# HongwenZhang/DaNet-DensePose2SMPL

Measured on AMD Instinct MI355X. Metric: images/sec fwd+bwd HRNet-W48+SMPL+IUV 256x256 bs32/GPU, higher is better.
Workload: dtype bf16; 1 GPU; full DaNet train step (HRNet-W48 + global and part-wise IUV heads + regressor nets + SMPL LBS (2 forward + 1 backward; the 2 label-side forwards belong to the untimed batch prologue) + IUV render + losses, fwd+bwd+Adam), 256x256, 32 img/GPU; convs bf16 MFMA fp32-acc, LBS/raster/losses fp32; global_batch=32, parallelism=dp1

## Files before the change

### danet-densepose2smpl_amd/_lib.py

```python
import ctypes
import os

_HERE = os.path.dirname(os.path.abspath(__file__))
LIB_PATH = os.environ.get('DANET_LIB') or os.path.join(_HERE, 'csrc', 'libdanet_hip.so')
_lib = None

c_f = ctypes.c_void_p
c_i = ctypes.c_int
c_sz = ctypes.c_size_t
c_fl = ctypes.c_float

_SIGNATURES = {
    'danet_version': (c_i, []),
    'danet_last_error': (ctypes.c_char_p, []),
    'danet_smpl_lbs_debug': (c_i, [c_f]),
    'danet_smpl_lbs_ctx_floats': (c_sz, [c_i]),
    'danet_smpl_lbs_fwd_ws_floats': (c_sz, [c_i, c_i, c_i]),
    'danet_smpl_lbs_bwd_ws_floats': (c_sz, [c_i, c_i, c_i]),
    'danet_smpl_lbs_ticket_words': (c_sz, [c_i]),
    'danet_smpl_lbs_forward': (c_i, [c_f, c_f, c_i] + [c_f] * 9 + [c_i] * 4 + [c_f] * 5 + [c_sz, c_f, c_f]),
    'danet_smpl_lbs_backward': (c_i, [c_f, c_f, c_i] + [c_f] * 7 + [c_i] * 4 + [c_f] * 7 + [c_sz, c_f, c_i, c_f]),
    'danet_smpl_lbs_backward_fused_ok': (c_i, [c_i, c_i, c_i]),
    'danet_iuv_raster_ws_bytes': (c_sz, [c_i, c_i, c_i]),
    'danet_iuv_raster_forward': (c_i, [c_f, c_f, c_i, c_i, c_f, c_i, c_f, c_f, c_i, c_fl, c_fl, c_i, c_f, c_f, c_f, c_f, c_sz, c_f]),
# ... 133 lines not shown


class BnBwdJob(ctypes.Structure):
    _fields_ = [(k, ctypes.c_void_p) for k in ('dy', 'x', 'y', 'gamma', 'saved', 'dx', 'dres', 'dparam', 'red', 'beta', 'mask')] + \
               [('M', ctypes.c_int64), ('C', c_i), ('red_state', c_i), ('relu', c_i), ('mask_mode', c_i)]


class GcnLayer(ctypes.Structure):
    _fields_ = [(k, ctypes.c_void_p) for k in ('W', 'bias', 'gamma', 'beta', 'running_mean', 'running_var')]


class GcnTailArgs(ctypes.Structure):
    _fields_ = [('x', ctypes.c_void_p), ('L', GcnLayer * 5)] + \
               [(k, ctypes.c_void_p) for k in ('A_r2p', 'A_p2r', 'A_mask', 'edge')] + \
               [('Wp', ctypes.c_void_p * 2), ('bp', ctypes.c_void_p * 2), ('Wc', ctypes.c_void_p * 2), ('bc', ctypes.c_void_p * 2)] + \
               [(k, ctypes.c_void_p) for k in ('mean_pose', 'ws', 'jr0', 'jp0', 'jp1', 'pose', 'g_jr0', 'g_jp0', 'g_jp1', 'g_pose', 'gx')] + \
               [('gW', ctypes.c_void_p * 5), ('gb', ctypes.c_void_p * 5), ('ggamma', ctypes.c_void_p * 5), ('gbeta', ctypes.c_void_p * 5),
                ('gedge', ctypes.c_void_p),
                ('gWp', ctypes.c_void_p * 2), ('gbp', ctypes.c_void_p * 2), ('gWc', ctypes.c_void_p * 2), ('gbc', ctypes.c_void_p * 2),
                ('scratch', ctypes.c_void_p), ('bar', ctypes.c_void_p), ('B', c_i), ('momentum', ctypes.c_float), ('eps', ctypes.c_float)]


class ConvJob(ctypes.Structure):
    _fields_ = [(k, ctypes.c_void_p) for k in ('x', 'wp', 'y', 'bn_sums', 'bn_x', 'bn_y', 'bn_saved', 'bn_red', 'addend')] + \
               [(k, c_i) for k in ('B', 'H', 'W', 'Cin', 'OH', 'OW', 'Cout', 'R', 'S', 'stride', 'pad', 'dil', 'groups', 'transposed', 'bn_gate')]


def exported_symbols():
    return list(_SIGNATURES)


KNOBS = {'c3_enable': 1, 'c3_mt': 2, 'c3_kw': 3, 'c3_blocks': 4, 'c3_want': 5, 'c3s_enable': 6, 'c3s_blocks': 7, 'c3s_kw': 8, 'c3s_want': 9,
         'pw': 10, 'pw_wgrad': 11, 'stem': 12, 'stem_dgrad': 13, 'c3a': 14, 'bn_block_bytes': 15,
         'c3s_balance': 16, 'c3s_tile_cost': 17, 'g3': 18}


class _Library(object):

    def __init__(self, cdll):
        self._cdll = cdll

    def __getattr__(self, name):
        return getattr(self._cdll, name)

    def knob(self, name, value=-1):
        return int(self._cdll.danet_knob(KNOBS[name], int(value)))

    def danet_conv3x3_set(self, enable, force_mt, force_kw, blocks, want_tiles):
        prev = self.knob('c3_enable', enable)
        if force_mt >= 0 and force_kw >= 0:
            self.knob('c3_mt', force_mt)
            self.knob('c3_kw', force_kw)
        self.knob('c3_blocks', blocks if blocks > 0 else -1)
        self.knob('c3_want', want_tiles)
        return prev

    def danet_conv3x3_stream_set(self, enable, blocks, kw, want_tiles):
        prev = self.knob('c3s_enable', enable)
        self.knob('c3s_blocks', blocks if blocks > 0 else -1)
        self.knob('c3s_kw', kw)
        self.knob('c3s_want', want_tiles)
        return prev

    def danet_conv_pw_set(self, enable):
        return self.knob('pw', enable)

    def danet_conv_pw_wgrad_set(self, enable):
# ... 68 lines not shown
```

### danet-densepose2smpl_amd/csrc/capi.hip

```cpp
#include "common.h"
#include "conv_common.h"

namespace danet {
char* last_error_buf() {
    static thread_local char buf[kErrLen] = {0};
    return buf;
}

namespace {
__global__ __launch_bounds__(256) void zero_kernel(unsigned* __restrict__ p, size_t n4, size_t tail0, size_t n) {
    uint4* const q = reinterpret_cast<uint4*>(p);
    for (size_t i = (size_t)blockIdx.x * 256 + threadIdx.x; i < n4; i += (size_t)gridDim.x * 256) q[i] = uint4{0u, 0u, 0u, 0u};
    for (size_t i = tail0 + (size_t)blockIdx.x * 256 + threadIdx.x; i < n; i += (size_t)gridDim.x * 256) p[i] = 0u;
}
}

hipError_t zero_async(void* p, size_t bytes, hipStream_t stream) {
    if (bytes == 0) return hipSuccess;
    if ((bytes & 3) || (reinterpret_cast<size_t>(p) & 3)) return hipErrorInvalidValue;
    const size_t n = bytes / 4;
    const bool al16 = (reinterpret_cast<size_t>(p) & 15) == 0;
    const size_t n4 = al16 ? n / 4 : 0, tail0 = n4 * 4;
    size_t blocks = ((al16 ? n4 : n) + 255) / 256;
    if (blocks > 2048) blocks = 2048;
    if (blocks < 1) blocks = 1;
    hipLaunchKernelGGL(zero_kernel, dim3((unsigned)blocks), dim3(256), 0, stream, (unsigned*)p, n4, tail0, n);
    return hipGetLastError();
}
}

extern "C" int danet_version(void) { return 100; }

extern "C" long danet_knob(int id, long value) {
    using namespace danet_conv;
    switch (id) {
        case DANET_KNOB_C3_ENABLE: case DANET_KNOB_C3_MT: case DANET_KNOB_C3_KW: case DANET_KNOB_C3_BLOCKS: case DANET_KNOB_C3_WANT:
            return conv3x3_knob(id, value);
        case DANET_KNOB_C3S_ENABLE: case DANET_KNOB_C3S_BLOCKS: case DANET_KNOB_C3S_KW: case DANET_KNOB_C3S_WANT:
        case DANET_KNOB_C3S_BALANCE: case DANET_KNOB_C3S_TILE_COST:
            return conv3x3s_knob(id, value);
        case DANET_KNOB_PW: return conv_pw_knob(value);
        case DANET_KNOB_PW_WGRAD: return conv_pw_wgrad_knob(value);
        case DANET_KNOB_STEM: return conv_stem_knob(value);
        case DANET_KNOB_STEM_DGRAD: return conv_stem_dgrad_knob(value);
        case DANET_KNOB_C3A: return conv3x3a_knob(value);
        case DANET_KNOB_G3: return conv_g3_knob(value);
        case DANET_KNOB_BN_BLOCK_BYTES: return bn_block_bytes_knob(value);
        default: return -1;
    }
}
extern "C" const char* danet_last_error(void) { return danet::last_error_buf(); }
```

### danet-densepose2smpl_amd/csrc/conv_common.h

```cpp
#pragma once
#include <hip/hip_runtime.h>

namespace danet_conv {

typedef unsigned short bf16_t;
typedef __attribute__((ext_vector_type(8))) __bf16 bf16x8;
typedef __attribute__((ext_vector_type(4))) float f32x4;

typedef __attribute__((ext_vector_type(2))) float f32x2_;
typedef __attribute__((ext_vector_type(2))) __bf16 bf16x2_;
__device__ inline unsigned f2bf_pk(float lo, float hi) {
    return __builtin_bit_cast(unsigned, __builtin_convertvector(f32x2_{lo, hi}, bf16x2_));
}
__device__ inline bf16_t f2bf(float f) { return (bf16_t)(f2bf_pk(f, 0.f) & 0xffffu); }
__device__ inline float bf2f(bf16_t h) { return __uint_as_float((unsigned)h << 16); }

constexpr int BN_NCOPY = 32;
#ifndef DANET_BN_NCOPY_DIV
#define DANET_BN_NCOPY_DIV 2
#endif
__host__ __device__ inline int bn_ncopy(int C) {
    const int n = (C <= 64 ? 32 : (C <= 128 ? 16 : (C <= 256 ? 8 : 4))) / DANET_BN_NCOPY_DIV;
    return n < 4 ? 4 : n;
}
// ... 34 lines not shown
    const bf16_t* addend;
    const BnApply* bna;
};


bool conv_fast_ok(const ConvP& p, bool vec8, int mt);
int conv_fast_launch(const ConvP& p, int mt, int nt, void* stream);
int conv_fast_launch_multi(const ConvP* ps, const int* mts, int n, int nt, void* stream);

bool conv_pw_ok(const ConvP& p, bool vec8);
int conv_pw_config(const ConvP& p);
int conv_pw_launch(const ConvP& p, void* stream);

struct WgJob { const void* x; const void* dy; float* dw; int B, H, W, Cin, OH, OW, Cout, R, S, stride, pad, dil, groups; };
bool conv_pw_wgrad_ok(const WgJob& j);
size_t conv_pw_wgrad_ws_floats(const WgJob* jobs, const int* idx, int cnt, long target);
int conv_pw_wgrad_launch(const WgJob* jobs, const int* idx, int cnt, float* ws, float beta, long target, void* stream);

bool conv_g3_ok(const ConvP& p, bool vec8);
int conv_g3_launch(const ConvP& p, void* stream);

bool conv3x3_ok(const ConvP& p, bool vec8);
int conv3x3_config(const ConvP& p, bool vec8, int nprob);
int conv3x3_launch(const ConvP* ps, int n, void* stream, bool dry = false);

int conv3x3s_launch(const ConvP* ps, int n, void* stream, bool dry);
bool conv3x3_stream_first();
int* conv3x3_debug_buffer();

long conv3x3_knob(int id, long value);
long conv3x3s_knob(int id, long value);
long conv_pw_knob(long value);
long conv_pw_wgrad_knob(long value);
long conv_stem_knob(long value);
long conv_stem_dgrad_knob(long value);
long conv3x3a_knob(long value);
long conv_g3_knob(long value);
long bn_block_bytes_knob(long value);

}
```

### danet-densepose2smpl_amd/csrc/conv_wgrad3x3.hip

```cpp
#include <cstdlib>
#include "common.h"
#include "conv_common.h"

namespace {

using namespace danet_conv;

constexpr int TH = 4, TW = 8;
constexpr int halo_h(int st) { return st * (TH - 1) + 3; }
constexpr int halo_w(int st) { return st * (TW - 1) + 3; }

struct Wg3P {
    const bf16_t* x; const bf16_t* dy; float* part;
    float* direct;
    int B, H, W, Cin, Cout, groups, Cin_g, Cout_g;
    int IH, IW;
    int tiles_h, tiles_w, msplit;
    long nchunks;
    long x_bytes, dy_bytes;
};

typedef __attribute__((ext_vector_type(2))) unsigned v2u;

__device__ inline v2u tr_read(unsigned lds_byte_addr) {
    v2u r;
    asm volatile("ds_read_b64_tr_b16 %0, %1" : "=v"(r) : "v"(lds_byte_addr) : "memory");
    return r;
}

template <int CT, int NI, int ST, int SM = 0>
__device__ __forceinline__ void wgrad3x3_body(const Wg3P& p, const int bx, const int by, const int bz)
{
    constexpr bool PAIR = SM != 0;
    constexpr int OS = SM ? SM : 4;
    constexpr int PHW = ST * (OS - 1) + 3;
    constexpr int IMH = SM ? TH / OS : 1, IMW = SM ? TW / OS : 1;
    constexpr int HH = SM ? IMH * PHW : halo_h(ST), HW = SM ? IMW * PHW : halo_w(ST);
    constexpr int HALF = SM ? (4 / OS) * PHW : ST * 4;
    constexpr int BCO = CT * 16, BCI = NI * 16;
    constexpr int PXY = BCO * 2, PXX = BCI * 2;
    extern __shared__ __attribute__((aligned(16))) unsigned char smem[];
    constexpr int YB = TH * TW * PXY, XB = HH * HW * PXX, BUF = YB + XB;

    const int t = threadIdx.x, lane = t & 63, wave = t >> 6;
    const int li = lane & 15, lg = lane >> 4;
    const int nci = (p.Cin_g + BCI - 1) / BCI;
    const int cib = by % nci, cob = by / nci;
    const int g = bz;
    const int co0 = cob * BCO, ci0 = cib * BCI;
    const bf16_t* const dyg = p.dy + (size_t)g * p.Cout_g + co0;
    const bf16_t* const xg = p.x + (size_t)g * p.Cin_g + ci0;

    constexpr int NPAIR = 9 * NI;
    constexpr int MAXP = (NPAIR + 3) / 4;
    f32x4 acc[MAXP][CT];
    unsigned boff[MAXP];
#pragma unroll
    for (int pi = 0; pi < MAXP; ++pi) {
#pragma unroll
        for (int ct = 0; ct < CT; ++ct) acc[pi][ct] = f32x4{0.f, 0.f, 0.f, 0.f};
        const int pair = min(wave + 4 * pi, NPAIR - 1);
        const int tap = pair / NI, ni = pair - tap * NI;
        const int r = tap / 3, s = tap - r * 3;
        const int hrow = SM ? (lg / OS) * PHW + ST * (lg % OS) + r : ST * lg + r;
        const int hcol = SM ? ((li >> 2) / OS) * PHW + ST * ((li >> 2) % OS) + s : ST * (li >> 2) + s;
        boff[pi] = (unsigned)((hrow * HW + hcol) * PXX + (ni * 16 + 4 * (li & 3)) * 2);
    }
    const unsigned aoff = (unsigned)((lg * TW + (li >> 2)) * PXY + (4 * (li & 3)) * 2);

    const int nchunks = (int)p.nchunks;
    const int per = (nchunks + p.msplit - 1) / p.msplit;
    const int c_begin = bx * per, c_end = min(nchunks, c_begin + per);

    constexpr int NPY = TH * TW * (BCO / 8), NPX = HH * HW * (BCI / 8);
    constexpr int NRY = (NPY + 255) / 256, NRX = (NPX + 255) / 256;
    constexpr int OOB = 0x7fffffff;
    const __amdgpu_buffer_rsrc_t yr = __builtin_amdgcn_make_buffer_rsrc(const_cast<bf16_t*>(dyg), 0, (int)p.dy_bytes, 0x00020000);
    const __amdgpu_buffer_rsrc_t xr = __builtin_amdgcn_make_buffer_rsrc(const_cast<bf16_t*>(xg), 0, (int)p.x_bytes, 0x00020000);
    int yrel[NRY], xrel[NRX], xhy[NRX], xhx[NRX];
#pragma unroll
    for (int u = 0; u < NRY; ++u) {
        const int pc = t + u * 256;
        const int c8 = pc % (BCO / 8), q = pc / (BCO / 8);
        const int ty = q / TW, tx = q % TW;
        const int ypix = SM ? ((ty / OS) * IMW + tx / OS) * (OS * OS) + (ty % OS) * OS + tx % OS : ty * p.W + tx;
        yrel[u] = (pc < NPY && co0 + c8 * 8 < p.Cout_g) ? (ypix * p.Cout + c8 * 8) * 2 : OOB;
    }
#pragma unroll
    for (int u = 0; u < NRX; ++u) {
        const int pc = t + u * 256;
        const int c8 = pc % (BCI / 8), q = pc / (BCI / 8);
        const bool live = pc < NPX && ci0 + c8 * 8 < p.Cin_g;
        if (PAIR) {
            const int hq = q / HW, img = (hq / PHW) * IMW + (q % HW) / PHW, hy = hq % PHW - 1, hc = (q % HW) % PHW - 1;
            const bool inside = live && (unsigned)hy < (unsigned)(OS * ST) && (unsigned)hc < (unsigned)(OS * ST);
            xrel[u] = ((img * (OS * OS * ST * ST) + hy * (OS * ST) + hc) * p.Cin + c8 * 8) * 2;
            xhy[u] = inside ? 1 : -100000;
            xhx[u] = 1;
        } else {
            xrel[u] = (((q / HW - 1) * p.IW + q % HW - 1) * p.Cin + c8 * 8) * 2;
            xhy[u] = live ? q / HW : -100000;
            xhx[u] = q % HW;
        }
    }
    int f_tw = c_begin % p.tiles_w, f_th = (c_begin / p.tiles_w) % p.tiles_h, f_b = c_begin / (p.tiles_w * p.tiles_h);
    uint4 ystage[NRY], xstage[NRX];

    auto fetch = [&]() {
        const int oh0 = f_th * TH, ow0 = f_tw * TW;
        const int pix0 = (f_b * p.H + oh0) * p.W + ow0;
        const int by = pix0 * p.Cout * 2, bx = ((f_b * p.IH + ST * oh0) * p.IW + ST * ow0) * p.Cin * 2;
#pragma unroll
        for (int u = 0; u < NRY; ++u)
            ystage[u] = __builtin_bit_cast(uint4, __builtin_amdgcn_raw_buffer_load_b128(yr, yrel[u] != OOB ? by + yrel[u] : OOB, 0, 0));
#pragma unroll
        for (int u = 0; u < NRX; ++u) {
            const bool ok = PAIR ? xhy[u] > 0
                                 : ((unsigned)(ST * oh0 - 1 + xhy[u]) < (unsigned)p.IH && (unsigned)(ST * ow0 - 1 + xhx[u]) < (unsigned)p.IW);
            xstage[u] = __builtin_bit_cast(uint4, __builtin_amdgcn_raw_buffer_load_b128(xr, ok ? bx + xrel[u] : OOB, 0, 0));
        }
        if (++f_tw == p.tiles_w) { f_tw = 0; if (++f_th == p.tiles_h) { f_th = 0; ++f_b; } }
    };
    auto commit = [&](int buf) {
        unsigned char* base = smem + buf * BUF;
#pragma unroll
        for (int u = 0; u < NRY; ++u)
            if (t + u * 256 < NPY) *reinterpret_cast<uint4*>(base + (size_t)(t + u * 256) * 16) = ystage[u];
#pragma unroll
        for (int u = 0; u < NRX; ++u)
            if (t + u * 256 < NPX) *reinterpret_cast<uint4*>(base + (size_t)(NPY + t + u * 256) * 16) = xstage[u];
    };

    if (c_begin < c_end) fetch();
    int buf = 0;
    for (int ch = c_begin; ch < c_end; ++ch) {
        commit(buf);
        __syncthreads();
        if (ch + 1 < c_end) fetch();
        const unsigned ybase = (unsigned)(buf * BUF), xbase = ybase + YB;
        v2u alo[CT], ahi[CT], blo[MAXP], bhi[MAXP];
#pragma unroll
        for (int ct = 0; ct < CT; ++ct) {
            alo[ct] = tr_read(ybase + aoff + ct * 32);
            ahi[ct] = tr_read(ybase + aoff + ct * 32 + 4 * PXY);
        }
#pragma unroll
        for (int pi = 0; pi < MAXP; ++pi) {
            blo[pi] = tr_read(xbase + boff[pi]);
            bhi[pi] = tr_read(xbase + boff[pi] + HALF * PXX);
        }
        asm volatile("s_waitcnt lgkmcnt(0)" ::: "memory");
        __builtin_amdgcn_sched_barrier(0);
        bf16x8 a[CT];
#pragma unroll
        for (int ct = 0; ct < CT; ++ct) {
            const uint4 raw = {alo[ct].x, alo[ct].y, ahi[ct].x, ahi[ct].y};
            a[ct] = __builtin_bit_cast(bf16x8, raw);
        }
#pragma unroll
        for (int pi = 0; pi < MAXP; ++pi) {
            const uint4 raw = {blo[pi].x, blo[pi].y, bhi[pi].x, bhi[pi].y};
            const bf16x8 bq = __builtin_bit_cast(bf16x8, raw);
#pragma unroll
            for (int ct = 0; ct < CT; ++ct)
                acc[pi][ct] = __builtin_amdgcn_mfma_f32_16x16x32_bf16(a[ct], bq, acc[pi][ct], 0, 0, 0);
        }
        buf ^= 1;
    }
    const int gsz = 9 * p.Cout_g * p.Cin_g;
    if (p.direct) {
        float* const dw = p.direct + (size_t)g * gsz;
#pragma unroll
        for (int pi = 0; pi < MAXP; ++pi) {
            const int pair = wave + 4 * pi;
            const int tap = pair / NI, ni = pair - tap * NI;
            const int cin = ci0 + ni * 16 + li;
            if (pair >= NPAIR || cin >= p.Cin_g) continue;
#pragma unroll
            for (int ct = 0; ct < CT; ++ct)
#pragma unroll
                for (int r = 0; r < 4; ++r) {
                    const int cout = co0 + ct * 16 + lg * 4 + r;
                    if (cout < p.Cout_g) dw[((size_t)cout * p.Cin_g + cin) * 9 + tap] = acc[pi][ct][r];
                }
        }
        return;
    }
    float* dst = p.part + ((size_t)bx * p.groups + g) * gsz;
#pragma unroll
    for (int pi = 0; pi < MAXP; ++pi) {
        const int pair = wave + 4 * pi;
        const int tap = pair / NI, ni = pair - tap * NI;
        const int cin = ci0 + ni * 16 + li;
        if (pair >= NPAIR || cin >= p.Cin_g) continue;
        float* row = dst + ((tap * p.Cout_g + co0 + lg * 4) * p.Cin_g + cin);
#pragma unroll
        for (int ct = 0; ct < CT; ++ct)
#pragma unroll
            for (int r = 0; r < 4; ++r)
                if (co0 + ct * 16 + lg * 4 + r < p.Cout_g) row[(ct * 16 + r) * p.Cin_g] = acc[pi][ct][r];
    }
}

template <int CT, int NI, int ST>
__global__ __launch_bounds__(256) void conv_wgrad3x3_kernel(Wg3P p)
{
    wgrad3x3_body<CT, NI, ST>(p, blockIdx.x, blockIdx.y, blockIdx.z);
}

constexpr int NPM = 20;
struct Wg3Multi { Wg3P p[NPM]; int start[NPM + 1]; int nyb[NPM]; int n; int xcd; };

template <int CT, int NI, int ST, int SM = 0>
__global__ __launch_bounds__(256) void conv_wgrad3x3_multi_kernel(Wg3Multi mp)
{
    int vb = (int)blockIdx.x;
    if (mp.xcd) {
        const int G = (int)gridDim.x, q = G >> 3, r = G & 7;
        const int x = vb & 7, slot = vb >> 3;
        vb = x * q + (x < r ? x : r) + slot;
    }
    int i = 0;
    while (i + 1 < mp.n && vb >= mp.start[i + 1]) ++i;
    const int l = vb - mp.start[i];
    const Wg3P& p = mp.p[i];
    const int bx = l % p.msplit, rest = l / p.msplit;
    wgrad3x3_body<CT, NI, ST, SM>(p, bx, rest % mp.nyb[i], rest / mp.nyb[i]);
}

struct Red3Multi { const float* part[NPM]; float* dw[NPM]; int G[NPM], Cout_g[NPM], Cin_g[NPM], msplit[NPM]; long start[NPM + 1]; int n; float beta; };

__global__ __launch_bounds__(256) void wgrad3x3_reduce_multi_kernel(Red3Multi rp)
{
    const long gidx = (long)blockIdx.x * 256 + threadIdx.x;
    if (gidx >= rp.start[rp.n]) return;
    int i = 0;
    while (i + 1 < rp.n && gidx >= rp.start[i + 1]) ++i;
    const long idx = gidx - rp.start[i], total = rp.start[i + 1] - rp.start[i];
    const float* part = rp.part[i];
    float s = 0.f;
    int sp = 0;
    for (; sp + 4 <= rp.msplit[i]; sp += 4) {
        const float v0 = part[(size_t)sp * total + idx], v1 = part[(size_t)(sp + 1) * total + idx];
        const float v2 = part[(size_t)(sp + 2) * total + idx], v3 = part[(size_t)(sp + 3) * total + idx];
        s += (v0 + v1) + (v2 + v3);
    }
    for (; sp < rp.msplit[i]; ++sp) s += part[(size_t)sp * total + idx];
    const int Cin_g = rp.Cin_g[i], Cout_g = rp.Cout_g[i];
    const int cin = (int)(idx % Cin_g);
    long rest = idx / Cin_g;
    const int cout = (int)(rest % Cout_g); rest /= Cout_g;
    const int tap = (int)(rest % 9), g = (int)(rest / 9);
    const size_t o = (((size_t)(g * Cout_g + cout)) * Cin_g + cin) * 9 + tap;
    float* dw = rp.dw[i];
    dw[o] = rp.beta != 0.f ? dw[o] * rp.beta + s : s;
}

__global__ __launch_bounds__(256) void wgrad3x3_reduce_kernel(const float* __restrict__ part, float* __restrict__ dw,
                                                               int G, int Cout_g, int Cin_g, int msplit, float beta)
{
    const long total = (long)G * Cout_g * Cin_g * 9;
    const long idx = (long)blockIdx.x * 256 + threadIdx.x;
    if (idx >= total) return;
    float s = 0.f;
    int sp = 0;
    for (; sp + 4 <= msplit; sp += 4) {
        const float v0 = part[(size_t)sp * total + idx], v1 = part[(size_t)(sp + 1) * total + idx];
        const float v2 = part[(size_t)(sp + 2) * total + idx], v3 = part[(size_t)(sp + 3) * total + idx];
        s += (v0 + v1) + (v2 + v3);
    }
    for (; sp < msplit; ++sp) s += part[(size_t)sp * total + idx];
    const int cin = (int)(idx % Cin_g);
    long rest = idx / Cin_g;
    const int cout = (int)(rest % Cout_g); rest /= Cout_g;
    const int tap = (int)(rest % 9), g = (int)(rest / 9);
    const size_t o = (((size_t)(g * Cout_g + cout)) * Cin_g + cin) * 9 + tap;
    dw[o] = beta != 0.f ? dw[o] * beta + s : s;
}

template <int CT, int NI, int ST>
int launch3(const Wg3P& p, hipStream_t st) {
    const int nco = (p.Cout_g + CT * 16 - 1) / (CT * 16), nci = (p.Cin_g + NI * 16 - 1) / (NI * 16);
    const size_t lds = 2 * (size_t)(TH * TW * CT * 32 + halo_h(ST) * halo_w(ST) * NI * 32);
    hipLaunchKernelGGL((conv_wgrad3x3_kernel<CT, NI, ST>), dim3(p.msplit, nco * nci, p.groups), dim3(256), lds, st, p);
    return 0;
}

inline int tiles3(int c) { return c <= 16 ? 1 : (c <= 32 ? 2 : ((c % 48 == 0 || c <= 48) ? 3 : 4)); }

}

extern "C" int danet_conv_wgrad3x3_ok(int H, int W, int Cin, int Cout, int R, int S, int stride, int pad, int dil, int groups) {
    static const bool no_s2 = getenv("DANET_NO_WGRAD3_S2") != nullptr;
    if (!(R == 3 && S == 3 && (stride == 1 || (stride == 2 && !no_s2)) && pad == 1 && dil == 1)) return 0;
    if (H % stride != 0 || W % stride != 0) return 0;
    return (H / stride) % TH == 0 && (W / stride) % TW == 0 && (Cin / groups) % 8 == 0 && (Cout / groups) % 8 == 0;
}

extern "C" int danet_conv_wgrad3x3_pair_ok(int B, int H, int W, int Cin, int Cout, int R, int S, int stride, int pad, int dil, int groups) {
    static const bool off = getenv("DANET_NO_WGRAD3_PAIR") != nullptr;
    if (off || !(R == 3 && S == 3 && (stride == 1 || stride == 2) && pad == 1 && dil == 1 && H == W && B > 0 && groups > 0)) return 0;
    if (!((H == 4 * stride && B % 2 == 0) || (H == 2 * stride && B % 8 == 0))) return 0;
    if (Cin % groups != 0 || Cout % groups != 0) return 0;
    const int ci = Cin / groups, co = Cout / groups;
    if (ci % 8 != 0 || co % 8 != 0) return 0;
    return 1;
}
static inline int wg3_small(int B, int H, int W, int stride) {
    if (!(stride == 1 || stride == 2) || H != W) return 0;
    if (H == 4 * stride && B % 2 == 0) return 4;
    if (H == 2 * stride && B % 8 == 0) return 2;
    return 0;
}
static inline bool wg3_is_pair(int B, int H, int W, int stride) { return wg3_small(B, H, W, stride) != 0; }

static void plan3(int B, int H, int W, int Cin, int Cout, int groups, int* ct, int* ni, int* msplit) {
    const int Cout_g = Cout / groups, Cin_g = Cin / groups;
    *ct = tiles3(Cout_g); *ni = tiles3(Cin_g);
    if (*ct == 4) *ct = 2;
    if (*ni == 4) *ni = 2;
    const long other = (long)((Cout_g + *ct * 16 - 1) / (*ct * 16)) * ((Cin_g + *ni * 16 - 1) / (*ni * 16)) * groups;
    const long nchunks = (long)B * (H / TH) * (W / TW);
// ... 111 lines not shown
        int msplit[NPM];
        plan_multi(jobs, idx, cnt, ct, ni, msplit);
        Wg3Multi mp; Red3Multi rp;
        static const bool xcd_order = getenv("DANET_WGRAD3_XCD") && atoi(getenv("DANET_WGRAD3_XCD")) != 0;
        mp.n = cnt; rp.n = cnt; rp.beta = beta; mp.xcd = xcd_order ? 1 : 0;
        mp.start[0] = 0; rp.start[0] = 0;
        for (int k = 0; k < cnt; ++k) {
            const Wg3Job& j = jobs[idx[k]];
            Wg3P& p = mp.p[k];
            static const bool no_direct = getenv("DANET_WGRAD3_NO_DIRECT") != nullptr;
            const bool direct = msplit[k] == 1 && beta == 0.f && !no_direct;
            p.x = (const bf16_t*)j.x; p.dy = (const bf16_t*)j.dy; p.part = (ws && !direct) ? ws + used : nullptr;
            p.direct = direct ? j.dw : nullptr;
            p.IH = j.H; p.IW = j.W;
            p.B = j.B; p.H = j.H / stride; p.W = j.W / stride; p.Cin = j.Cin; p.Cout = j.Cout; p.groups = j.groups;
            if (pair) { p.B = j.B / (sm == 4 ? 2 : 8); p.H = 4; p.W = 8; p.IH = 4 * stride; p.IW = 8 * stride; }
            p.Cin_g = j.Cin / j.groups; p.Cout_g = j.Cout / j.groups;
            p.tiles_h = p.H / TH; p.tiles_w = p.W / TW;
            p.nchunks = (long)p.B * p.tiles_h * p.tiles_w;
            p.x_bytes = (long)j.B * j.H * j.W * j.Cin * 2; p.dy_bytes = (long)j.B * (j.H / stride) * (j.W / stride) * j.Cout * 2;
            p.msplit = msplit[k];
            const int nyb = ((p.Cout_g + ct * 16 - 1) / (ct * 16)) * ((p.Cin_g + ni * 16 - 1) / (ni * 16));
            mp.nyb[k] = nyb;
            mp.start[k + 1] = mp.start[k] + msplit[k] * nyb * j.groups;
            const long total = (long)j.Cout * p.Cin_g * 9;
            rp.part[k] = p.part; rp.dw[k] = j.dw; rp.G[k] = j.groups; rp.Cout_g[k] = p.Cout_g; rp.Cin_g[k] = p.Cin_g; rp.msplit[k] = msplit[k];
            rp.start[k + 1] = rp.start[k] + (direct ? 0 : total);
            if (!direct || !ws) used += (size_t)msplit[k] * total;
            if (ws && !(p.x_bytes < (1L << 31) && p.dy_bytes < (1L << 31)))
                return danet::fail(DANET_ERR_ARG, "conv_wgrad3x3_multi: tensors of 2 GB or more are not supported");
        }
        if (!ws) continue;
        if (used > ws_floats) return danet::fail(DANET_ERR_WORKSPACE, "conv_wgrad3x3_multi: workspace too small");
        const int phw = stride * ((sm ? sm : 4) - 1) + 3;
        const size_t lds = 2 * (size_t)(TH * TW * ct * 32 + (sm ? (TH / sm) * phw * (TW / sm) * phw : halo_h(stride) * halo_w(stride)) * ni * 32);
        const dim3 grid((unsigned)mp.start[cnt]);
        if (pair) {
#define W3P(a, b) if (ct == a && ni == b) { \
            if (stride == 1 && sm == 4) hipLaunchKernelGGL((conv_wgrad3x3_multi_kernel<a, b, 1, 4>), grid, dim3(256), lds, st, mp); \
            else if (stride == 2 && sm == 4) hipLaunchKernelGGL((conv_wgrad3x3_multi_kernel<a, b, 2, 4>), grid, dim3(256), lds, st, mp); \
            else if (stride == 1) hipLaunchKernelGGL((conv_wgrad3x3_multi_kernel<a, b, 1, 2>), grid, dim3(256), lds, st, mp); \
            else hipLaunchKernelGGL((conv_wgrad3x3_multi_kernel<a, b, 2, 2>), grid, dim3(256), lds, st, mp); } else
            W3P(2, 2) W3P(2, 3) W3P(3, 2) W3P(3, 3) W3P(1, 1) W3P(1, 2) W3P(2, 1) W3P(1, 3) W3P(3, 1)
            return danet::fail(DANET_ERR_ARG, "conv_wgrad3x3_multi: no pair-mode kernel for tiles %dx%d", ct, ni);
#undef W3P
        } else
#define W3M(a, b) if (ct == a && ni == b) { \
            if (stride == 1) hipLaunchKernelGGL((conv_wgrad3x3_multi_kernel<a, b, 1>), grid, dim3(256), lds, st, mp); \
            else hipLaunchKernelGGL((conv_wgrad3x3_multi_kernel<a, b, 2>), grid, dim3(256), lds, st, mp); } else
        W3M(1, 1) W3M(1, 2) W3M(1, 3) W3M(2, 1) W3M(2, 2) W3M(2, 3) W3M(3, 1) W3M(3, 2) W3M(3, 3)
        return danet::fail(DANET_ERR_ARG, "conv_wgrad3x3_multi: no kernel for tiles %dx%d", ct, ni);
#undef W3M
        DANET_CHECK_LAUNCH("conv_wgrad3x3_multi_kernel");
        if (rp.start[cnt] > 0) {
            hipLaunchKernelGGL(wgrad3x3_reduce_multi_kernel, dim3((unsigned)danet::cdiv(rp.start[cnt], 256)), dim3(256), 0, st, rp);
            DANET_CHECK_LAUNCH("wgrad3x3_reduce_multi_kernel");
        }
    }
    if (need_out) *need_out = used;
    return DANET_OK;
}

extern "C" size_t danet_conv_wgrad3x3_multi_ws_floats(const void* jobs, int n)
{
    size_t need = 0;
    if (!jobs || n <= 0) return 0;
    multi_foreach_launch((const Wg3Job*)jobs, n, nullptr, 0, 0.f, nullptr, &need);
    return need;
}

extern "C" int danet_conv_wgrad3x3_multi(const void* jobs, int n, float* ws, size_t ws_floats, float beta, void* stream)
{
    DANET_ENTER();
    DANET_CHECK_ARG(jobs && n > 0 && ws, "conv_wgrad3x3_multi: bad arguments");
    const Wg3Job* jb = (const Wg3Job*)jobs;
    for (int i = 0; i < n; ++i)
        DANET_CHECK_ARG(jb[i].x && jb[i].dy && jb[i].dw && jb[i].B > 0 &&
                        (danet_conv_wgrad3x3_ok(jb[i].H, jb[i].W, jb[i].Cin, jb[i].Cout, 3, 3, jb[i].stride, 1, 1, jb[i].groups) ||
                         danet_conv_wgrad3x3_pair_ok(jb[i].B, jb[i].H, jb[i].W, jb[i].Cin, jb[i].Cout, 3, 3, jb[i].stride, 1, 1, jb[i].groups)),
                        "conv_wgrad3x3_multi: job %d is not a supported 3x3 problem", i);
    return multi_foreach_launch(jb, n, ws, ws_floats, beta, (hipStream_t)stream, nullptr);
}
// ... 1 lines not shown
```

### include/danet_hip.h

```cpp
#ifndef DANET_HIP_H
#define DANET_HIP_H

#include <stddef.h>
#include <stdint.h>

#ifdef __cplusplus
extern "C" {
#endif

#define DANET_OK 0
#define DANET_ERR_ARG (-1)
#define DANET_ERR_HIP (-2)
#define DANET_ERR_WORKSPACE (-3)

int danet_version(void);
const char* danet_last_error(void);

size_t danet_smpl_lbs_ctx_floats(int B);
size_t danet_smpl_lbs_fwd_ws_floats(int B, int V, int NE);
size_t danet_smpl_lbs_bwd_ws_floats(int B, int V, int NB);
size_t danet_smpl_lbs_ticket_words(int B);

int danet_smpl_lbs_forward(const float* betas, const float* rotmats, int B,
                           const float* v_template, const float* shapedirs, const float* posedirs,
// ... 106 lines not shown
int danet_conv_pack_weights_padded(const float* w, void* wp, int Cout, int Cin_g, int R, int S, int groups,
                                   int mode, int chunk, int src_Cout_g, int src_Cin_g, void* stream);
long danet_conv_pack_job_fill_padded(void* job_host, const float* w, void* wp, long start, long bstart,
                                     int Cout, int Cin_g, int R, int S, int groups, int mode, int chunk, int src_Cout_g, int src_Cin_g);
size_t danet_conv_pack_job_bytes(void);
long danet_conv_pack_job_bricks(int Cout, int Cin_g, int R, int S, int groups, int mode, int chunk);
long danet_conv_pack_job_fill(void* job_host, const float* w, void* wp, long start, long bstart,
                              int Cout, int Cin_g, int R, int S, int groups, int mode, int chunk);
int danet_conv_pack_weights_batched(const void* jobs_dev, int njobs, long total_elems, long total_bricks, void* stream);
int danet_conv_f32(int mode, const float* a, const float* b, const float* bias, float* out,
                   int B, int H, int W, int Cin, int OH, int OW, int Cout, int R, int S, int stride, int pad, int dil, int groups,
                   void* stream);
size_t danet_conv_f32m_packed_elems(int Cout_gp, int Cin_gp, int R, int S, int groups, int mode);
int danet_conv_f32m_pack_weights(const float* w, float* wp, int Cout, int Cin_g, int R, int S, int groups, int mode,
                                 int Cout_gp, int Cin_gp, void* stream);
int danet_conv_f32m_ok(int B, int H, int W, int Cin, int OH, int OW, int Cout, int R, int S, int stride, int pad, int dil,
                       int groups, int transposed);
int danet_conv_f32m_forward(const float* x, const float* wp, const float* bias, float* y,
                            int B, int H, int W, int Cin, int OH, int OW, int Cout, int R, int S, int stride, int pad, int dil,
                            int groups, int transposed, int relu, void* stream);
size_t danet_conv_f32m_wgrad_ws_floats(int B, int H, int W, int Cin, int OH, int OW, int Cout, int R, int S, int stride, int pad,
                                       int dil, int groups, int Cout_real, int Cin_g_real);
int danet_conv_f32m_wgrad(const float* x, const float* dy, float* dw, float* ws,
                          int B, int H, int W, int Cin, int OH, int OW, int Cout, int R, int S, int stride, int pad, int dil, int groups,
                          int Cout_real, int Cin_g_real, void* stream);
int danet_conv_forward_multi_ok(const void* jobs, int n);
int danet_conv_bn_forward_multi_ok(const void* jobs, int n, const void* bn_jobs, void* bar);
int danet_conv_bn_forward_multi(const void* jobs, int n, const void* bn_jobs, float momentum, float eps, void* bar, int* fused, void* stream);
int danet_conv_forward_multi_kernel(const void* jobs, int n);
enum { DANET_KNOB_C3_ENABLE = 1, DANET_KNOB_C3_MT = 2, DANET_KNOB_C3_KW = 3, DANET_KNOB_C3_BLOCKS = 4, DANET_KNOB_C3_WANT = 5,
       DANET_KNOB_C3S_ENABLE = 6, DANET_KNOB_C3S_BLOCKS = 7, DANET_KNOB_C3S_KW = 8, DANET_KNOB_C3S_WANT = 9,
       DANET_KNOB_PW = 10, DANET_KNOB_PW_WGRAD = 11, DANET_KNOB_STEM = 12, DANET_KNOB_STEM_DGRAD = 13, DANET_KNOB_C3A = 14,
       DANET_KNOB_BN_BLOCK_BYTES = 15, DANET_KNOB_C3S_BALANCE = 16, DANET_KNOB_C3S_TILE_COST = 17,
       DANET_KNOB_G3 = 18  };
long danet_knob(int id, long value);
int danet_conv3x3_stream_plan(int B, int H, int W, int Cin, int Cout, int nprob);
size_t danet_conv3x3_stream_table_bytes(void);
int danet_conv3x3_stream_tables(void* workspace, size_t bytes);
int danet_conv_stem_ok(int B, int H, int W, int Cin, int OH, int OW, int Cout, int R, int S, int stride, int pad, int dil, int groups);
int danet_conv_stem_forward(const void* x, const void* wp, void* y, int B, int H, int W, int Cin, int OH, int OW, int Cout,
                            float* bn_sums, void* stream);
int danet_conv_stem_dgrad_ok(int B, int H, int W, int Cin, int OH, int OW, int Cout, int R, int S, int stride, int pad, int dil, int groups);
int danet_conv_stem_dgrad(const void* dy, const void* wp, void* dx, int B, int H, int W, int Cin, int OH, int OW, int Cout,
                          const void* bn_x, const void* bn_y, const float* bn_saved, float* bn_red, void* stream);
int danet_conv3x3a_ok(int B, int H, int W, int Cin, int Cout, int R, int S, int stride, int pad, int dil, int groups);
int danet_conv3x3a(const void* x, const void* wp, void* y, int B, int H, int W, int transposed, float* bn_sums,
                   const void* bn_x, const void* bn_y, const float* bn_saved, float* bn_red, int bn_gate, const void* addend, void* stream);
void danet_conv3x3_debug(int* dev_buf);
int danet_conv_forward_multi(const void* jobs, int n, void* stream);
int danet_conv_forward_kernel(int B, int H, int W, int Cin, int OH, int OW, int Cout, int R, int S,
                              int stride, int pad, int dil, int groups, int transposed, int out_fp32);
int danet_conv_forward(const void* x, const void* wp, const float* bias, void* y,
                       int B, int H, int W, int Cin, int OH, int OW, int Cout,
                       int R, int S, int stride, int pad, int dil, int groups, int transposed,
                       int relu, int out_fp32, float* bn_sums,
                       const void* bn_x, const void* bn_y, const float* bn_saved, float* bn_red, const void* addend,
                       int bn_gate, void* stream);
int danet_conv_wgrad3x3_ok(int H, int W, int Cin, int Cout, int R, int S, int stride, int pad, int dil, int groups);
int danet_conv_wgrad3x3_pair_ok(int B, int H, int W, int Cin, int Cout, int R, int S, int stride, int pad, int dil, int groups);
size_t danet_conv_wgrad3x3_ws_floats(int B, int H, int W, int Cin, int Cout, int groups, int stride);
size_t danet_conv_wgrad3x3_multi_ws_floats(const void* jobs, int n);
size_t danet_conv_wgrad_multi_ws_floats(const void* jobs, int n);
size_t danet_conv_wgrad_multi_ws_zero_from(const void* jobs, int n);
int danet_conv_wgrad_multi(const void* jobs, int n, float* ws, size_t ws_floats, float beta, void* stream);
int danet_conv_wgrad3x3_multi(const void* jobs, int n, float* ws, size_t ws_floats, float beta, void* stream);
int danet_conv_wgrad3x3_kernel_id(int B, int H, int W, int Cin, int Cout, int groups, int stride);
int danet_conv_wgrad3x3(const void* x, const void* dy, float* dw, float* ws, size_t ws_floats,
// ... 75 lines not shown
```

Before: 1336 images/sec.

## Pipeline 3x3 wgrad tile loads with direct-to-LDS buffer DMA and multi-stage ring

Adds a pipelined path for the 3x3 weight-gradient kernels. Tiles are loaded with buffer_load ... lds instructions straight into a 3 or 4 slot LDS ring, using per-wave vmcnt waits and one barrier per step, in place of the register-staged double buffer. This removes the register round trip and the separate LDS store, and keeps more loads in flight. It is on by default, can be switched off through an env var or knob, and uses more LDS, which may lower occupancy.

New measurement: 1335 images/sec (median of 6 runs). About the same (-0.1%).

```diff
diff --git a/danet-densepose2smpl_amd/_lib.py b/danet-densepose2smpl_amd/_lib.py
--- a/danet-densepose2smpl_amd/_lib.py
+++ b/danet-densepose2smpl_amd/_lib.py
@@ -189,7 +189,7 @@
 
 KNOBS = {'c3_enable': 1, 'c3_mt': 2, 'c3_kw': 3, 'c3_blocks': 4, 'c3_want': 5, 'c3s_enable': 6, 'c3s_blocks': 7, 'c3s_kw': 8, 'c3s_want': 9,
          'pw': 10, 'pw_wgrad': 11, 'stem': 12, 'stem_dgrad': 13, 'c3a': 14, 'bn_block_bytes': 15,
-         'c3s_balance': 16, 'c3s_tile_cost': 17, 'g3': 18}
+         'c3s_balance': 16, 'c3s_tile_cost': 17, 'g3': 18, 'wgrad3_pipe': 19}
 
 
 class _Library(object):
diff --git a/danet-densepose2smpl_amd/csrc/capi.hip b/danet-densepose2smpl_amd/csrc/capi.hip
--- a/danet-densepose2smpl_amd/csrc/capi.hip
+++ b/danet-densepose2smpl_amd/csrc/capi.hip
@@ -41,6 +41,7 @@
             return conv3x3s_knob(id, value);
         case DANET_KNOB_PW: return conv_pw_knob(value);
         case DANET_KNOB_PW_WGRAD: return conv_pw_wgrad_knob(value);
+        case DANET_KNOB_WGRAD3_PIPE: return conv_wgrad3x3_pipe_knob(value);
         case DANET_KNOB_STEM: return conv_stem_knob(value);
         case DANET_KNOB_STEM_DGRAD: return conv_stem_dgrad_knob(value);
         case DANET_KNOB_C3A: return conv3x3a_knob(value);
diff --git a/danet-densepose2smpl_amd/csrc/conv_common.h b/danet-densepose2smpl_amd/csrc/conv_common.h
--- a/danet-densepose2smpl_amd/csrc/conv_common.h
+++ b/danet-densepose2smpl_amd/csrc/conv_common.h
@@ -90,6 +90,7 @@
 long conv3x3s_knob(int id, long value);
 long conv_pw_knob(long value);
 long conv_pw_wgrad_knob(long value);
+long conv_wgrad3x3_pipe_knob(long value);
 long conv_stem_knob(long value);
 long conv_stem_dgrad_knob(long value);
 long conv3x3a_knob(long value);
diff --git a/danet-densepose2smpl_amd/csrc/conv_wgrad3x3.hip b/danet-densepose2smpl_amd/csrc/conv_wgrad3x3.hip
--- a/danet-densepose2smpl_amd/csrc/conv_wgrad3x3.hip
+++ b/danet-densepose2smpl_amd/csrc/conv_wgrad3x3.hip
@@ -9,6 +9,41 @@
 constexpr int TH = 4, TW = 8;
 constexpr int halo_h(int st) { return st * (TH - 1) + 3; }
 constexpr int halo_w(int st) { return st * (TW - 1) + 3; }
+
+template <int CT, int NI, int ST, int SM>
+struct Wg3Geo {
+    static constexpr int OS = SM ? SM : 4;
+    static constexpr int PHW = ST * (OS - 1) + 3;
+    static constexpr int IMH = SM ? TH / OS : 1, IMW = SM ? TW / OS : 1;
+    static constexpr int HH = SM ? IMH * PHW : halo_h(ST), HW = SM ? IMW * PHW : halo_w(ST);
+    static constexpr int BCO = CT * 16, BCI = NI * 16;
+    static constexpr int PXY = BCO * 2, PXX = BCI * 2;
+    static constexpr int YB = TH * TW * PXY, XB = HH * HW * PXX, BUF = YB + XB;
+    static constexpr int NPY = TH * TW * (BCO / 8), NPX = HH * HW * (BCI / 8);
+    static constexpr int NS = 12 * BUF <= 160 * 1024 ? 4 : 3;
+    static_assert(NPY % 64 == 0, "dY tile = whole 1 KB copies");
+};
+template <int CT, int NI, int ST, int SM, bool PIPE>
+constexpr size_t wg3_lds_bytes() { using G = Wg3Geo<CT, NI, ST, SM>; return (size_t)(PIPE ? G::NS : 2) * G::BUF; }
+
+typedef __attribute__((ext_vector_type(4))) int i32x4;
+typedef __attribute__((address_space(3))) void* lds_ptr_t;
+
+__device__ __forceinline__ void dma16(unsigned lds_addr, int voff, const i32x4& desc) {
+    asm volatile("s_mov_b32 m0, %0\n\ts_nop 0\n\tbuffer_load_dwordx4 %1, %2, 0 offen lds" :: "s"(lds_addr), "v"(voff), "s"(desc) : "memory");
+}
+__device__ inline i32x4 raw_desc(const void* base, int bytes) {
+    const unsigned long long a = reinterpret_cast<unsigned long long>(base);
+    return i32x4{__builtin_amdgcn_readfirstlane((int)(unsigned)a), __builtin_amdgcn_readfirstlane((int)((a >> 32) & 0xffffu)),
+                 __builtin_amdgcn_readfirstlane(bytes), 0x00020000};
+}
+template <int N>
+__device__ __forceinline__ void vm_wait() { static_assert(N >= 0 && N <= 63, "vmcnt"); asm volatile("s_waitcnt vmcnt(%0)" :: "n"(N) : "memory"); }
+__device__ inline void lds_barrier() {
+    __builtin_amdgcn_fence(__ATOMIC_RELEASE, "workgroup", "local");
+    __builtin_amdgcn_s_barrier();
+    __builtin_amdgcn_fence(__ATOMIC_ACQUIRE, "workgroup", "local");
+}
 
 struct Wg3P {
     const bf16_t* x; const bf16_t* dy; float* part;
@@ -28,19 +63,16 @@
     return r;
 }
 
-template <int CT, int NI, int ST, int SM = 0>
+template <int CT, int NI, int ST, int SM = 0, bool PIPE = false>
 __device__ __forceinline__ void wgrad3x3_body(const Wg3P& p, const int bx, const int by, const int bz)
 {
+    using G = Wg3Geo<CT, NI, ST, SM>;
     constexpr bool PAIR = SM != 0;
-    constexpr int OS = SM ? SM : 4;
-    constexpr int PHW = ST * (OS - 1) + 3;
-    constexpr int IMH = SM ? TH / OS : 1, IMW = SM ? TW / OS : 1;
-    constexpr int HH = SM ? IMH * PHW : halo_h(ST), HW = SM ? IMW * PHW : halo_w(ST);
+    constexpr int OS = G::OS, PHW = G::PHW, IMW = G::IMW, HW = G::HW;
     constexpr int HALF = SM ? (4 / OS) * PHW : ST * 4;
-    constexpr int BCO = CT * 16, BCI = NI * 16;
-    constexpr int PXY = BCO * 2, PXX = BCI * 2;
+    constexpr int BCO = G::BCO, BCI = G::BCI, PXY = G::PXY, PXX = G::PXX;
     extern __shared__ __attribute__((aligned(16))) unsigned char smem[];
-    constexpr int YB = TH * TW * PXY, XB = HH * HW * PXX, BUF = YB + XB;
+    constexpr int YB = G::YB, BUF = G::BUF;
 
     const int t = threadIdx.x, lane = t & 63, wave = t >> 6;
     const int li = lane & 15, lg = lane >> 4;
@@ -72,72 +104,37 @@
     const int per = (nchunks + p.msplit - 1) / p.msplit;
     const int c_begin = bx * per, c_end = min(nchunks, c_begin + per);
 
-    constexpr int NPY = TH * TW * (BCO / 8), NPX = HH * HW * (BCI / 8);
-    constexpr int NRY = (NPY + 255) / 256, NRX = (NPX + 255) / 256;
+    constexpr int NPY = G::NPY, NPX = G::NPX;
     constexpr int OOB = 0x7fffffff;
-    const __amdgpu_buffer_rsrc_t yr = __builtin_amdgcn_make_buffer_rsrc(const_cast<bf16_t*>(dyg), 0, (int)p.dy_bytes, 0x00020000);
-    const __amdgpu_buffer_rsrc_t xr = __builtin_amdgcn_make_buffer_rsrc(const_cast<bf16_t*>(xg), 0, (int)p.x_bytes, 0x00020000);
-    int yrel[NRY], xrel[NRX], xhy[NRX], xhx[NRX];
-#pragma unroll
-    for (int u = 0; u < NRY; ++u) {
-        const int pc = t + u * 256;
+    auto ypiece = [&](int pc) -> int {
         const int c8 = pc % (BCO / 8), q = pc / (BCO / 8);
         const int ty = q / TW, tx = q % TW;
         const int ypix = SM ? ((ty / OS) * IMW + tx / OS) * (OS * OS) + (ty % OS) * OS + tx % OS : ty * p.W + tx;
-        yrel[u] = (pc < NPY && co0 + c8 * 8 < p.Cout_g) ? (ypix * p.Cout + c8 * 8) * 2 : OOB;
-    }
-#pragma unroll
-    for (int u = 0; u < NRX; ++u) {
-        const int pc = t + u * 256;
+        return (pc < NPY && co0 + c8 * 8 < p.Cout_g) ? (ypix * p.Cout + c8 * 8) * 2 : OOB;
+    };
+    auto xpiece = [&](int pc, int& xrel, int& xhy, int& xhx) {
         const int c8 = pc % (BCI / 8), q = pc / (BCI / 8);
         const bool live = pc < NPX && ci0 + c8 * 8 < p.Cin_g;
         if (PAIR) {
             const int hq = q / HW, img = (hq / PHW) * IMW + (q % HW) / PHW, hy = hq % PHW - 1, hc = (q % HW) % PHW - 1;
             const bool inside = live && (unsigned)hy < (unsigned)(OS * ST) && (unsigned)hc < (unsigned)(OS * ST);
-            xrel[u] = ((img * (OS * OS * ST * ST) + hy * (OS * ST) + hc) * p.Cin + c8 * 8) * 2;
-            xhy[u] = inside ? 1 : -100000;
-            xhx[u] = 1;
+            xrel = ((img * (OS * OS * ST * ST) + hy * (OS * ST) + hc) * p.Cin + c8 * 8) * 2;
+            xhy = inside ? 1 : -100000;
+            xhx = 1;
         } else {
-            xrel[u] = (((q / HW - 1) * p.IW + q % HW - 1) * p.Cin + c8 * 8) * 2;
-            xhy[u] = live ? q / HW : -100000;
-            xhx[u] = q % HW;
-        }
-    }
+            xrel = (((q / HW - 1) * p.IW + q % HW - 1) * p.Cin + c8 * 8) * 2;
+            xhy = live ? q / HW : -100000;
+            xhx = q % HW;
+        }
+    };
+    auto x_ok = [&](int oh0, int ow0, int xhy, int xhx) -> bool {
+        return PAIR ? xhy > 0 : ((unsigned)(ST * oh0 - 1 + xhy) < (unsigned)p.IH && (unsigned)(ST * ow0 - 1 + xhx) < (unsigned)p.IW);
+    };
     int f_tw = c_begin % p.tiles_w, f_th = (c_begin / p.tiles_w) % p.tiles_h, f_b = c_begin / (p.tiles_w * p.tiles_h);
-    uint4 ystage[NRY], xstage[NRX];
-
-    auto fetch = [&]() {
-        const int oh0 = f_th * TH, ow0 = f_tw * TW;
-        const int pix0 = (f_b * p.H + oh0) * p.W + ow0;
-        const int by = pix0 * p.Cout * 2, bx = ((f_b * p.IH + ST * oh0) * p.IW + ST * ow0) * p.Cin * 2;
-#pragma unroll
-        for (int u = 0; u < NRY; ++u)
-            ystage[u] = __builtin_bit_cast(uint4, __builtin_amdgcn_raw_buffer_load_b128(yr, yrel[u] != OOB ? by + yrel[u] : OOB, 0, 0));
-#pragma unroll
-        for (int u = 0; u < NRX; ++u) {
-            const bool ok = PAIR ? xhy[u] > 0
-                                 : ((unsigned)(ST * oh0 - 1 + xhy[u]) < (unsigned)p.IH && (unsigned)(ST * ow0 - 1 + xhx[u]) < (unsigned)p.IW);
-            xstage[u] = __builtin_bit_cast(uint4, __builtin_amdgcn_raw_buffer_load_b128(xr, ok ? bx + xrel[u] : OOB, 0, 0));
-        }
-        if (++f_tw == p.tiles_w) { f_tw = 0; if (++f_th == p.tiles_h) { f_th = 0; ++f_b; } }
-    };
-    auto commit = [&](int buf) {
-        unsigned char* base = smem + buf * BUF;
-#pragma unroll
-        for (int u = 0; u < NRY; ++u)
-            if (t + u * 256 < NPY) *reinterpret_cast<uint4*>(base + (size_t)(t + u * 256) * 16) = ystage[u];
-#pragma unroll
-        for (int u = 0; u < NRX; ++u)
-            if (t + u * 256 < NPX) *reinterpret_cast<uint4*>(base + (size_t)(NPY + t + u * 256) * 16) = xstage[u];
-    };
-
-    if (c_begin < c_end) fetch();
-    int buf = 0;
-    for (int ch = c_begin; ch < c_end; ++ch) {
-        commit(buf);
-        __syncthreads();
-        if (ch + 1 < c_end) fetch();
-        const unsigned ybase = (unsigned)(buf * BUF), xbase = ybase + YB;
+    auto advance = [&]() { if (++f_tw == p.tiles_w) { f_tw = 0; if (++f_th == p.tiles_h) { f_th = 0; ++f_b; } } };
+
+    auto compute = [&](unsigned ybase) {
+        const unsigned xbase = ybase + YB;
         v2u alo[CT], ahi[CT], blo[MAXP], bhi[MAXP];
 #pragma unroll
         for (int ct = 0; ct < CT; ++ct) {
@@ -165,7 +162,101 @@
             for (int ct = 0; ct < CT; ++ct)
                 acc[pi][ct] = __builtin_amdgcn_mfma_f32_16x16x32_bf16(a[ct], bq, acc[pi][ct], 0, 0, 0);
         }
-        buf ^= 1;
+    };
+
+    if constexpr (!PIPE) {
+        constexpr int NRY = (NPY + 255) / 256, NRX = (NPX + 255) / 256;
+        const __amdgpu_buffer_rsrc_t yr = __builtin_amdgcn_make_buffer_rsrc(const_cast<bf16_t*>(dyg), 0, (int)p.dy_bytes, 0x00020000);
+        const __amdgpu_buffer_rsrc_t xr = __builtin_amdgcn_make_buffer_rsrc(const_cast<bf16_t*>(xg), 0, (int)p.x_bytes, 0x00020000);
+        int yrel[NRY], xrel[NRX], xhy[NRX], xhx[NRX];
+#pragma unroll
+        for (int u = 0; u < NRY; ++u) yrel[u] = ypiece(t + u * 256);
+#pragma unroll
+        for (int u = 0; u < NRX; ++u) xpiece(t + u * 256, xrel[u], xhy[u], xhx[u]);
+        uint4 ystage[NRY], xstage[NRX];
+
+        auto fetch = [&]() {
+            const int oh0 = f_th * TH, ow0 = f_tw * TW;
+            const int pix0 = (f_b * p.H + oh0) * p.W + ow0;
+            const int by = pix0 * p.Cout * 2, bx = ((f_b * p.IH + ST * oh0) * p.IW + ST * ow0) * p.Cin * 2;
+#pragma unroll
+            for (int u = 0; u < NRY; ++u)
+                ystage[u] = __builtin_bit_cast(uint4, __builtin_amdgcn_raw_buffer_load_b128(yr, yrel[u] != OOB ? by + yrel[u] : OOB, 0, 0));
+#pragma unroll
+            for (int u = 0; u < NRX; ++u)
+                xstage[u] = __builtin_bit_cast(uint4, __builtin_amdgcn_raw_buffer_load_b128(xr, x_ok(oh0, ow0, xhy[u], xhx[u]) ? bx + xrel[u] : OOB, 0, 0));
+            advance();
+        };
+        auto commit = [&](int buf) {
+            unsigned char* base = smem + buf * BUF;
+#pragma unroll
+            for (int u = 0; u < NRY; ++u)
+                if (t + u * 256 < NPY) *reinterpret_cast<uint4*>(base + (size_t)(t + u * 256) * 16) = ystage[u];
+#pragma unroll
+            for (int u = 0; u < NRX; ++u)
+                if (t + u * 256 < NPX) *reinterpret_cast<uint4*>(base + (size_t)(NPY + t + u * 256) * 16) = xstage[u];
+        };
+
+        if (c_begin < c_end) fetch();
+        int buf = 0;
+        for (int ch = c_begin; ch < c_end; ++ch) {
+            commit(buf);
+            __syncthreads();
+            if (ch + 1 < c_end) fetch();
+            compute((unsigned)(buf * BUF));
+            buf ^= 1;
+        }
+    } else {
+        constexpr int NIY = NPY / 64, NIT = NIY + (NPX + 63) / 64;
+        constexpr int KHI = (NIT + 3) / 4, NS = G::NS;
+        static_assert(KHI * (NS - 2) <= 63, "vmcnt");
+        const int wv = __builtin_amdgcn_readfirstlane(wave);
+        const bool khi = wv < NIT - 4 * (KHI - 1);
+        const i32x4 yd = raw_desc(dyg, (int)p.dy_bytes), xd = raw_desc(xg, (int)p.x_bytes);
+        int rel[KHI], hy[KHI], hx[KHI];
+        unsigned live = 0;
+#pragma unroll
+        for (int r = 0; r < KHI; ++r) {
+            const int j = wv + 4 * r, pc = j * 64 + lane;
+            if (j < NIY) {
+                rel[r] = ypiece(pc);
+                hy[r] = rel[r] != OOB ? 1 : -100000;
+                hx[r] = 1;
+            } else {
+                xpiece(pc - NPY, rel[r], hy[r], hx[r]);
+            }
+            if (j < NIT && pc < NPY + NPX) live |= 1u << r;
+        }
+        const unsigned lds0 = (unsigned)(unsigned long long)(lds_ptr_t)smem;
+        auto issue = [&](int slot) {
+            const int oh0 = f_th * TH, ow0 = f_tw * TW;
+            const int by = ((f_b * p.H + oh0) * p.W + ow0) * p.Cout * 2, bx = ((f_b * p.IH + ST * oh0) * p.IW + ST * ow0) * p.Cin * 2;
+            const unsigned dst = lds0 + (unsigned)(slot * BUF);
+#pragma unroll
+            for (int r = 0; r < KHI; ++r) {
+                const int j = wv + 4 * r;
+                if (j < NIT) {
+                    const bool isy = j < NIY;
+                    const int voff = x_ok(oh0, ow0, hy[r], hx[r]) ? (isy ? by : bx) + rel[r] : OOB;
+                    if ((live >> r) & 1u) dma16(__builtin_amdgcn_readfirstlane(dst + (unsigned)j * 1024u), voff, isy ? yd : xd);
+                }
+            }
+            advance();
+        };
+
+        const int n = c_end - c_begin;
+#pragma unroll
+        for (int k = 0; k < NS - 1; ++k)
+            if (k < n) issue(k);
+        int slot = 0;
+        for (int i = 0; i < n; ++i) {
+            if (i + NS - 2 < n) { if (khi) vm_wait<KHI * (NS - 2)>(); else vm_wait<(KHI - 1) * (NS - 2)>(); }
+            else vm_wait<0>();
+            lds_barrier();
+            if (i + NS - 1 < n) issue(slot == 0 ? NS - 1 : slot - 1);
+            compute(lds0 + (unsigned)(slot * BUF));
+            slot = slot + 1 == NS ? 0 : slot + 1;
+        }
     }
     const int gsz = 9 * p.Cout_g * p.Cin_g;
     if (p.direct) {
@@ -202,16 +293,16 @@
     }
 }
 
-template <int CT, int NI, int ST>
+template <int CT, int NI, int ST, bool PIPE>
 __global__ __launch_bounds__(256) void conv_wgrad3x3_kernel(Wg3P p)
 {
-    wgrad3x3_body<CT, NI, ST>(p, blockIdx.x, blockIdx.y, blockIdx.z);
+    wgrad3x3_body<CT, NI, ST, 0, PIPE>(p, blockIdx.x, blockIdx.y, blockIdx.z);
 }
 
 constexpr int NPM = 20;
 struct Wg3Multi { Wg3P p[NPM]; int start[NPM + 1]; int nyb[NPM]; int n; int xcd; };
 
-template <int CT, int NI, int ST, int SM = 0>
+template <int CT, int NI, int ST, int SM, bool PIPE>
 __global__ __launch_bounds__(256) void conv_wgrad3x3_multi_kernel(Wg3Multi mp)
 {
     int vb = (int)blockIdx.x;
@@ -225,7 +316,7 @@
     const int l = vb - mp.start[i];
     const Wg3P& p = mp.p[i];
     const int bx = l % p.msplit, rest = l / p.msplit;
-    wgrad3x3_body<CT, NI, ST, SM>(p, bx, rest % mp.nyb[i], rest / mp.nyb[i]);
+    wgrad3x3_body<CT, NI, ST, SM, PIPE>(p, bx, rest % mp.nyb[i], rest / mp.nyb[i]);
 }
 
 struct Red3Multi { const float* part[NPM]; float* dw[NPM]; int G[NPM], Cout_g[NPM], Cin_g[NPM], msplit[NPM]; long start[NPM + 1]; int n; float beta; };
@@ -278,16 +369,31 @@
     dw[o] = beta != 0.f ? dw[o] * beta + s : s;
 }
 
+bool g_wg3_pipe = !(getenv("DANET_WGRAD3_PIPE") && atoi(getenv("DANET_WGRAD3_PIPE")) == 0);
+
 template <int CT, int NI, int ST>
 int launch3(const Wg3P& p, hipStream_t st) {
     const int nco = (p.Cout_g + CT * 16 - 1) / (CT * 16), nci = (p.Cin_g + NI * 16 - 1) / (NI * 16);
-    const size_t lds = 2 * (size_t)(TH * TW * CT * 32 + halo_h(ST) * halo_w(ST) * NI * 32);
-    hipLaunchKernelGGL((conv_wgrad3x3_kernel<CT, NI, ST>), dim3(p.msplit, nco * nci, p.groups), dim3(256), lds, st, p);
+    const dim3 grid(p.msplit, nco * nci, p.groups);
+    if (g_wg3_pipe) hipLaunchKernelGGL((conv_wgrad3x3_kernel<CT, NI, ST, true>), grid, dim3(256), (wg3_lds_bytes<CT, NI, ST, 0, true>()), st, p);
+    else hipLaunchKernelGGL((conv_wgrad3x3_kernel<CT, NI, ST, false>), grid, dim3(256), (wg3_lds_bytes<CT, NI, ST, 0, false>()), st, p);
     return 0;
 }
 
+template <int CT, int NI, int ST, int SM>
+void launch_multi(const Wg3Multi& mp, dim3 grid, hipStream_t st) {
+    if (g_wg3_pipe) hipLaunchKernelGGL((conv_wgrad3x3_multi_kernel<CT, NI, ST, SM, true>), grid, dim3(256), (wg3_lds_bytes<CT, NI, ST, SM, true>()), st, mp);
+    else hipLaunchKernelGGL((conv_wgrad3x3_multi_kernel<CT, NI, ST, SM, false>), grid, dim3(256), (wg3_lds_bytes<CT, NI, ST, SM, false>()), st, mp);
+}
+
 inline int tiles3(int c) { return c <= 16 ? 1 : (c <= 32 ? 2 : ((c % 48 == 0 || c <= 48) ? 3 : 4)); }
 
+}
+
+long danet_conv::conv_wgrad3x3_pipe_knob(long enable) {
+    const long prev = g_wg3_pipe ? 1 : 0;
+    if (enable >= 0) g_wg3_pipe = enable != 0;
+    return prev;
 }
 
 extern "C" int danet_conv_wgrad3x3_ok(int H, int W, int Cin, int Cout, int R, int S, int stride, int pad, int dil, int groups) {
@@ -465,22 +571,20 @@
         }
         if (!ws) continue;
         if (used > ws_floats) return danet::fail(DANET_ERR_WORKSPACE, "conv_wgrad3x3_multi: workspace too small");
-        const int phw = stride * ((sm ? sm : 4) - 1) + 3;
-        const size_t lds = 2 * (size_t)(TH * TW * ct * 32 + (sm ? (TH / sm) * phw * (TW / sm) * phw : halo_h(stride) * halo_w(stride)) * ni * 32);
         const dim3 grid((unsigned)mp.start[cnt]);
         if (pair) {
 #define W3P(a, b) if (ct == a && ni == b) { \
-            if (stride == 1 && sm == 4) hipLaunchKernelGGL((conv_wgrad3x3_multi_kernel<a, b, 1, 4>), grid, dim3(256), lds, st, mp); \
-            else if (stride == 2 && sm == 4) hipLaunchKernelGGL((conv_wgrad3x3_multi_kernel<a, b, 2, 4>), grid, dim3(256), lds, st, mp); \
-            else if (stride == 1) hipLaunchKernelGGL((conv_wgrad3x3_multi_kernel<a, b, 1, 2>), grid, dim3(256), lds, st, mp); \
-            else hipLaunchKernelGGL((conv_wgrad3x3_multi_kernel<a, b, 2, 2>), grid, dim3(256), lds, st, mp); } else
+            if (stride == 1 && sm == 4) launch_multi<a, b, 1, 4>(mp, grid, st); \
+            else if (stride == 2 && sm == 4) launch_multi<a, b, 2, 4>(mp, grid, st); \
+            else if (stride == 1) launch_multi<a, b, 1, 2>(mp, grid, st); \
+            else launch_multi<a, b, 2, 2>(mp, grid, st); } else
             W3P(2, 2) W3P(2, 3) W3P(3, 2) W3P(3, 3) W3P(1, 1) W3P(1, 2) W3P(2, 1) W3P(1, 3) W3P(3, 1)
             return danet::fail(DANET_ERR_ARG, "conv_wgrad3x3_multi: no pair-mode kernel for tiles %dx%d", ct, ni);
 #undef W3P
         } else
 #define W3M(a, b) if (ct == a && ni == b) { \
-            if (stride == 1) hipLaunchKernelGGL((conv_wgrad3x3_multi_kernel<a, b, 1>), grid, dim3(256), lds, st, mp); \
-            else hipLaunchKernelGGL((conv_wgrad3x3_multi_kernel<a, b, 2>), grid, dim3(256), lds, st, mp); } else
+            if (stride == 1) launch_multi<a, b, 1, 0>(mp, grid, st); \
+            else launch_multi<a, b, 2, 0>(mp, grid, st); } else
         W3M(1, 1) W3M(1, 2) W3M(1, 3) W3M(2, 1) W3M(2, 2) W3M(2, 3) W3M(3, 1) W3M(3, 2) W3M(3, 3)
         return danet::fail(DANET_ERR_ARG, "conv_wgrad3x3_multi: no kernel for tiles %dx%d", ct, ni);
 #undef W3M
diff --git a/include/danet_hip.h b/include/danet_hip.h
--- a/include/danet_hip.h
+++ b/include/danet_hip.h
@@ -162,7 +162,8 @@
        DANET_KNOB_C3S_ENABLE = 6, DANET_KNOB_C3S_BLOCKS = 7, DANET_KNOB_C3S_KW = 8, DANET_KNOB_C3S_WANT = 9,
        DANET_KNOB_PW = 10, DANET_KNOB_PW_WGRAD = 11, DANET_KNOB_STEM = 12, DANET_KNOB_STEM_DGRAD = 13, DANET_KNOB_C3A = 14,
        DANET_KNOB_BN_BLOCK_BYTES = 15, DANET_KNOB_C3S_BALANCE = 16, DANET_KNOB_C3S_TILE_COST = 17,
-       DANET_KNOB_G3 = 18  };
+       DANET_KNOB_G3 = 18 ,
+       DANET_KNOB_WGRAD3_PIPE = 19  };
 long danet_knob(int id, long value);
 int danet_conv3x3_stream_plan(int B, int H, int W, int Cin, int Cout, int nprob);
 size_t danet_conv3x3_stream_table_bytes(void);
```
